# zijinxuxu/PDFNet

Hardware: AMD Instinct MI355X
Metric: train-step images/sec @256x256 RGB-D B=32 (higher is better)
Workload: dtype f32

## Files before the change

pdfnet_amd/csrc/winograd.hip:

```cpp
#include "common.h"
#include <cstdio>

int pdf_internal_batched_gemm(const float* A, const float* B, float* C, int batch, long gsA, long gsB, long gsC, int M, int N, int K, hipStream_t s);

template <bool FLIP>
__global__ __launch_bounds__(256) void wino_weight_kernel(const float* __restrict__ w, float* __restrict__ U, int Cout, int Cin) {
    const int N = FLIP ? Cin : Cout, K = FLIP ? Cout : Cin;
    const long total = (long)N * K;
    for (long i = blockIdx.x * 256L + threadIdx.x; i < total; i += (long)gridDim.x * 256) {
        const int n = (int)(i / K), k = (int)(i - (long)n * K);
        float g[3][3];
#pragma unroll
        for (int a = 0; a < 3; ++a)
#pragma unroll
            for (int b = 0; b < 3; ++b)
                g[a][b] = FLIP ? w[(((long)k * 3 + (2 - a)) * 3 + (2 - b)) * Cin + n] : w[(((long)n * 3 + a) * 3 + b) * Cin + k];
        float t[4][3];
#pragma unroll
        for (int b = 0; b < 3; ++b) {
            t[0][b] = g[0][b];
            t[1][b] = 0.5f * (g[0][b] + g[1][b] + g[2][b]);
            t[2][b] = 0.5f * (g[0][b] - g[1][b] + g[2][b]);
            t[3][b] = g[2][b];
        }
#pragma unroll
        for (int a = 0; a < 4; ++a) {
            const float u0 = t[a][0], u1 = 0.5f * (t[a][0] + t[a][1] + t[a][2]), u2 = 0.5f * (t[a][0] - t[a][1] + t[a][2]), u3 = t[a][2];
            U[(long)(a * 4 + 0) * total + i] = u0;
            U[(long)(a * 4 + 1) * total + i] = u1;
            U[(long)(a * 4 + 2) * total + i] = u2;
            U[(long)(a * 4 + 3) * total + i] = u3;
        }
    }
}

__global__ __launch_bounds__(256) void wino_input_kernel(const float* __restrict__ x, int ldx, float* __restrict__ V, int N, int H, int W, int C) {
    const int C4 = C >> 2, TW = W >> 1, TH = H >> 1;
    const long T = (long)N * TH * TW, total = T * C4;
    const long plane = T * C;
    for (long i = blockIdx.x * 256L + threadIdx.x; i < total; i += (long)gridDim.x * 256) {
        const long t = i / C4;
        const int c = (int)(i - t * C4) * 4;
        const int n = (int)(t / (TH * TW)), r = (int)(t - (long)n * TH * TW), ty = r / TW, tx = r - ty * TW;
        float4 d[4][4];
#pragma unroll
        for (int a = 0; a < 4; ++a) {
            const int iy = 2 * ty - 1 + a;
#pragma unroll
            for (int b = 0; b < 4; ++b) {
                const int ix = 2 * tx - 1 + b;
                d[a][b] = (iy >= 0 && iy < H && ix >= 0 && ix < W) ? *reinterpret_cast<const float4*>(x + (((long)n * H + iy) * W + ix) * ldx + c)
                                                                   : make_float4(0.f, 0.f, 0.f, 0.f);
            }
        }
        float4 s[4][4];
#pragma unroll
        for (int b = 0; b < 4; ++b) {
#define WSUB(p, q) make_float4(p.x - q.x, p.y - q.y, p.z - q.z, p.w - q.w)
#define WADD(p, q) make_float4(p.x + q.x, p.y + q.y, p.z + q.z, p.w + q.w)
            s[0][b] = WSUB(d[0][b], d[2][b]);
            s[1][b] = WADD(d[1][b], d[2][b]);
            s[2][b] = WSUB(d[2][b], d[1][b]);
            s[3][b] = WSUB(d[1][b], d[3][b]);
        }
#pragma unroll
        for (int a = 0; a < 4; ++a) {
            const float4 v0 = WSUB(s[a][0], s[a][2]), v1 = WADD(s[a][1], s[a][2]), v2 = WSUB(s[a][2], s[a][1]), v3 = WSUB(s[a][1], s[a][3]);
            float* o = V + t * C + c;
            *reinterpret_cast<float4*>(o + (long)(a * 4 + 0) * plane) = v0;
            *reinterpret_cast<float4*>(o + (long)(a * 4 + 1) * plane) = v1;
            *reinterpret_cast<float4*>(o + (long)(a * 4 + 2) * plane) = v2;
            *reinterpret_cast<float4*>(o + (long)(a * 4 + 3) * plane) = v3;
        }
    }
}

__global__ __launch_bounds__(256) void wino_output_kernel(const float* __restrict__ Mx, const float* __restrict__ bias, float* __restrict__ y, int ldy,
                                                          int N, int H, int W, int Co, int act, int accum) {
    const int C4 = Co >> 2, TW = W >> 1, TH = H >> 1;
    const long T = (long)N * TH * TW, total = T * C4;
    const long plane = T * Co;
    for (long i = blockIdx.x * 256L + threadIdx.x; i < total; i += (long)gridDim.x * 256) {
        const long t = i / C4;
        const int c = (int)(i - t * C4) * 4;
        const int n = (int)(t / (TH * TW)), r = (int)(t - (long)n * TH * TW), ty = r / TW, tx = r - ty * TW;
        float4 m[4][4];
        const float* p = Mx + t * Co + c;
#pragma unroll
        for (int a = 0; a < 4; ++a)
#pragma unroll
            for (int b = 0; b < 4; ++b) m[a][b] = *reinterpret_cast<const float4*>(p + (long)(a * 4 + b) * plane);
        float4 s[2][4];
#pragma unroll
        for (int b = 0; b < 4; ++b) {
            s[0][b] = WADD(WADD(m[0][b], m[1][b]), m[2][b]);
            s[1][b] = WSUB(WSUB(m[1][b], m[2][b]), m[3][b]);
        }
        const float4 bv = bias != nullptr ? *reinterpret_cast<const float4*>(bias + c) : make_float4(0.f, 0.f, 0.f, 0.f);
#pragma unroll
        for (int a = 0; a < 2; ++a) {
            float4 o[2];
            o[0] = WADD(WADD(s[a][0], s[a][1]), s[a][2]);
            o[1] = WSUB(WSUB(s[a][1], s[a][2]), s[a][3]);
#pragma unroll
            for (int b = 0; b < 2; ++b) {
                float4 v = WADD(o[b], bv);
                if (act == 1) v = make_float4(fmaxf(v.x, 0.f), fmaxf(v.y, 0.f), fmaxf(v.z, 0.f), fmaxf(v.w, 0.f));
                else if (act == 2) v = make_float4(v.x > 0.f ? v.x : 0.1f * v.x, v.y > 0.f ? v.y : 0.1f * v.y, v.z > 0.f ? v.z : 0.1f * v.z, v.w > 0.f ? v.w : 0.1f * v.w);
                float* q = y + (((long)n * H + 2 * ty + a) * W + 2 * tx + b) * ldy + c;
                if (accum) { const float4 e = *reinterpret_cast<const float4*>(q); v = WADD(v, e); }
                *reinterpret_cast<float4*>(q) = v;
            }
        }
    }
}
#undef WSUB
#undef WADD

template <bool FLIP, bool X3>
__global__ __launch_bounds__(256) void wino4_weight_kernel(const float* __restrict__ w, float* __restrict__ U, int Cout, int Cin) {
    const int N = FLIP ? Cin : Cout, K = FLIP ? Cout : Cin;
    const long total = (long)N * K;
    for (long i = blockIdx.x * 256L + threadIdx.x; i < total; i += (long)gridDim.x * 256) {
        const int n = (int)(i / K), k = (int)(i - (long)n * K);
        float g[3][3];
#pragma unroll
        for (int a = 0; a < 3; ++a)
#pragma unroll
            for (int b = 0; b < 3; ++b)
                g[a][b] = FLIP ? w[(((long)k * 3 + (2 - a)) * 3 + (2 - b)) * Cin + n] : w[(((long)n * 3 + a) * 3 + b) * Cin + k];
        float t[6][3];
#pragma unroll
        for (int b = 0; b < 3; ++b) {
            const float g0 = g[0][b], g1 = g[1][b], g2 = g[2][b];
            t[0][b] = g0 * 0.25f;
            t[1][b] = -(g0 + g1 + g2) * (1.f / 6.f);
            t[2][b] = -(g0 - g1 + g2) * (1.f / 6.f);
            t[3][b] = g0 * (1.f / 24.f) + g1 * (1.f / 12.f) + g2 * (1.f / 6.f);
            t[4][b] = g0 * (1.f / 24.f) - g1 * (1.f / 12.f) + g2 * (1.f / 6.f);
            t[5][b] = g2;
        }
#pragma unroll
        for (int a = 0; a < 6; ++a) {
            const float g0 = t[a][0], g1 = t[a][1], g2 = t[a][2];
            const float u[6] = {g0 * 0.25f, -(g0 + g1 + g2) * (1.f / 6.f), -(g0 - g1 + g2) * (1.f / 6.f),
                                g0 * (1.f / 24.f) + g1 * (1.f / 12.f) + g2 * (1.f / 6.f), g0 * (1.f / 24.f) - g1 * (1.f / 12.f) + g2 * (1.f / 6.f), g2};
#pragma unroll
            for (int b = 0; b < 6; ++b) {
                if constexpr (X3) {
                    unsigned h, m, l;
                    pdf_x3_split2(u[b], 0.f, h, m, l);
                    unsigned short* o = reinterpret_cast<unsigned short*>(U) + (long)(a * 6 + b) * total + i;
                    o[0] = (unsigned short)h; o[36 * total] = (unsigned short)m; o[72 * total] = (unsigned short)l;
                } else U[(long)(a * 6 + b) * total + i] = u[b];
            }
        }
    }
}
__device__ __forceinline__ void wino4_bt(float2 (&v)[6]) {
    const float2 d0 = v[0], d1 = v[1], d2 = v[2], d3 = v[3], d4 = v[4], d5 = v[5];
#define W4(e) make_float2(e(x), e(y))
#define E0(c) 4.f * d0.c - 5.f * d2.c + d4.c
#define E1(c) -4.f * (d1.c + d2.c) + d3.c + d4.c
#define E2(c) 4.f * (d1.c - d2.c) - d3.c + d4.c
#define E3(c) 2.f * (d3.c - d1.c) - d2.c + d4.c
#define E4(c) 2.f * (d1.c - d3.c) - d2.c + d4.c
#define E5(c) 4.f * d1.c - 5.f * d3.c + d5.c
    v[0] = W4(E0); v[1] = W4(E1); v[2] = W4(E2); v[3] = W4(E3); v[4] = W4(E4); v[5] = W4(E5);
#undef E0
#undef E1
#undef E2
#undef E3
#undef E4
#undef E5
}
template <bool X3>
__global__ __launch_bounds__(256) void wino4_input_kernel(const float* __restrict__ x, int ldx, float* __restrict__ V, int N, int H, int W, int C) {
    const int C2 = C >> 1, TW = W >> 2, TH = H >> 2;
    const long T = (long)N * TH * TW, total = T * C2;
    const long plane = T * C;
    for (long i = blockIdx.x * 256L + threadIdx.x; i < total; i += (long)gridDim.x * 256) {
        const long t = i / C2;
        const int c = (int)(i - t * C2) * 2;
        const int n = (int)(t / (TH * TW)), r = (int)(t - (long)n * TH * TW), ty = r / TW, tx = r - ty * TW;
        float2 d[6][6];
#pragma unroll
        for (int a = 0; a < 6; ++a) {
            const int iy = 4 * ty - 1 + a;
#pragma unroll
            for (int b = 0; b < 6; ++b) {
                const int ix = 4 * tx - 1 + b;
                d[a][b] = (iy >= 0 && iy < H && ix >= 0 && ix < W) ? *reinterpret_cast<const float2*>(x + (((long)n * H + iy) * W + ix) * ldx + c) : make_float2(0.f, 0.f);
            }
        }
#pragma unroll
        for (int b = 0; b < 6; ++b) {
            float2 col[6] = {d[0][b], d[1][b], d[2][b], d[3][b], d[4][b], d[5][b]};
            wino4_bt(col);
#pragma unroll
            for (int a = 0; a < 6; ++a) d[a][b] = col[a];
        }
        float* o = V + t * C + c;
#pragma unroll
        for (int a = 0; a < 6; ++a) {
            wino4_bt(d[a]);
#pragma unroll
            for (int b = 0; b < 6; ++b) {
                if constexpr (X3) pdf_x3_store2(reinterpret_cast<unsigned short*>(V), t * C + c + (long)(a * 6 + b) * plane, 36 * plane, d[a][b].x, d[a][b].y);
                else *reinterpret_cast<float2*>(o + (long)(a * 6 + b) * plane) = d[a][b];
            }
        }
    }
}
__global__ __launch_bounds__(256) void wino4_output_kernel(const float* __restrict__ Mx, const float* __restrict__ bias, float* __restrict__ y, int ldy,
                                                           int N, int H, int W, int Co, int act, int accum) {
    const int C2 = Co >> 1, TW = W >> 2, TH = H >> 2;
    const long T = (long)N * TH * TW, total = T * C2;
    const long plane = T * Co;
    for (long i = blockIdx.x * 256L + threadIdx.x; i < total; i += (long)gridDim.x * 256) {
        const long t = i / C2;
        const int c = (int)(i - t * C2) * 2;
        const int n = (int)(t / (TH * TW)), r = (int)(t - (long)n * TH * TW), ty = r / TW, tx = r - ty * TW;
        const float* p = Mx + t * Co + c;
        float2 s[4][6];
#pragma unroll
        for (int b = 0; b < 6; ++b) {
            float2 m[6];
#pragma unroll
            for (int a = 0; a < 6; ++a) m[a] = *reinterpret_cast<const float2*>(p + (long)(a * 6 + b) * plane);
#define O0(c) m[0].c + m[1].c + m[2].c + m[3].c + m[4].c
#define O1(c) m[1].c - m[2].c + 2.f * (m[3].c - m[4].c)
#define O2(c) m[1].c + m[2].c + 4.f * (m[3].c + m[4].c)
#define O3(c) m[1].c - m[2].c + 8.f * (m[3].c - m[4].c) + m[5].c
            s[0][b] = W4(O0); s[1][b] = W4(O1); s[2][b] = W4(O2); s[3][b] = W4(O3);
        }
        const float2 bv = bias != nullptr ? *reinterpret_cast<const float2*>(bias + c) : make_float2(0.f, 0.f);
#pragma unroll
        for (int a = 0; a < 4; ++a) {
            const float2* m = s[a];
            float2 o[4] = {W4(O0), W4(O1), W4(O2), W4(O3)};
#pragma unroll
            for (int b = 0; b < 4; ++b) {
                float2 v = make_float2(o[b].x + bv.x, o[b].y + bv.y);
                if (act == 1) v = make_float2(fmaxf(v.x, 0.f), fmaxf(v.y, 0.f));
                else if (act == 2) v = make_float2(v.x > 0.f ? v.x : 0.1f * v.x, v.y > 0.f ? v.y : 0.1f * v.y);
                float* q = y + (((long)n * H + 4 * ty + a) * W + 4 * tx + b) * ldy + c;
                if (accum) { const float2 e = *reinterpret_cast<const float2*>(q); v.x += e.x; v.y += e.y; }
                *reinterpret_cast<float2*>(q) = v;
            }
        }
#undef O0
#undef O1
#undef O2
#undef O3
#undef W4
    }
}

template <bool X3>
__global__ __launch_bounds__(256) void wino4_dy_kernel(const float* __restrict__ dy, int lddy, float* __restrict__ Yh, int N, int H, int W, int Co) {
    const int C2 = Co >> 1, TW = W >> 2, TH = H >> 2;
    const long T = (long)N * TH * TW, total = T * C2;
    const long plane = T * Co;
    for (long i = blockIdx.x * 256L + threadIdx.x; i < total; i += (long)gridDim.x * 256) {
        const long t = i / C2;
        const int c = (int)(i - t * C2) * 2;
        const int n = (int)(t / (TH * TW)), r = (int)(t - (long)n * TH * TW), ty = r / TW, tx = r - ty * TW;
        float2 d[4][4];
#pragma unroll
        for (int a = 0; a < 4; ++a)
#pragma unroll
            for (int b = 0; b < 4; ++b) d[a][b] = *reinterpret_cast<const float2*>(dy + (((long)n * H + 4 * ty + a) * W + 4 * tx + b) * lddy + c);
        float2 u[6][4];
#pragma unroll
        for (int b = 0; b < 4; ++b) {
#define A2(e) make_float2(e(x), e(y))
#define P0(k) d[0][b].k
#define P1(k) d[0][b].k + d[1][b].k + d[2][b].k + d[3][b].k
#define P2(k) d[0][b].k - d[1][b].k + d[2][b].k - d[3][b].k
#define P3(k) d[0][b].k + 2.f * d[1][b].k + 4.f * d[2][b].k + 8.f * d[3][b].k
#define P4(k) d[0][b].k - 2.f * d[1][b].k + 4.f * d[2][b].k - 8.f * d[3][b].k
#define P5(k) d[3][b].k
            u[0][b] = A2(P0); u[1][b] = A2(P1); u[2][b] = A2(P2); u[3][b] = A2(P3); u[4][b] = A2(P4); u[5][b] = A2(P5);
#undef P0
#undef P1
#undef P2
#undef P3
#undef P4
#undef P5
        }
        float* o = Yh + t * Co + c;
#pragma unroll
        for (int a = 0; a < 6; ++a) {
            const float2 e0 = u[a][0], e1 = u[a][1], e2 = u[a][2], e3 = u[a][3];
#define Q0(k) e0.k
#define Q1(k) e0.k + e1.k + e2.k + e3.k
#define Q2(k) e0.k - e1.k + e2.k - e3.k
#define Q3(k) e0.k + 2.f * e1.k + 4.f * e2.k + 8.f * e3.k
#define Q4(k) e0.k - 2.f * e1.k + 4.f * e2.k - 8.f * e3.k
#define Q5(k) e3.k
            const float2 q[6] = {A2(Q0), A2(Q1), A2(Q2), A2(Q3), A2(Q4), A2(Q5)};
#pragma unroll
            for (int b = 0; b < 6; ++b) {
                if constexpr (X3) pdf_x3_store2(reinterpret_cast<unsigned short*>(Yh), t * Co + c + (long)(a * 6 + b) * plane, 36 * plane, q[b].x, q[b].y);
                else *reinterpret_cast<float2*>(o + (long)(a * 6 + b) * plane) = q[b];
            }
#undef Q0
#undef Q1
#undef Q2
#undef Q3
#undef Q4
#undef Q5
#undef A2
        }
    }
}
__global__ __launch_bounds__(256) void wino4_slab_sum_kernel(float* __restrict__ slab, int splits, long total4) {
    for (long i = blockIdx.x * 256L + threadIdx.x; i < 36 * total4; i += (long)gridDim.x * 256) {
        const long p = i / total4, e = i - p * total4;
        float4* base = reinterpret_cast<float4*>(slab) + p * splits * total4 + e;
        float4 v = base[0];
        for (int y = 1; y < splits; ++y) { const float4 w = base[(long)y * total4]; v.x += w.x; v.y += w.y; v.z += w.z; v.w += w.w; }
        base[0] = v;
    }
}
__global__ __launch_bounds__(256) void wino4_wgrad_out_kernel(const float* __restrict__ slab, int splits, float* __restrict__ dw, int Co, int Ci, int accumulate) {
    const long total = (long)Co * Ci;
    for (long i = blockIdx.x * 256L + threadIdx.x; i < total; i += (long)gridDim.x * 256) {
        const int n = (int)(i / Ci), c = (int)(i - (long)n * Ci);
        float u[6][6];
#pragma unroll
        for (int p = 0; p < 36; ++p) u[p / 6][p % 6] = slab[(long)p * splits * total + i];
        {
        float t[3][6];
#pragma unroll
        for (int b = 0; b < 6; ++b) {
            t[0][b] = 0.25f * u[0][b] - (1.f / 6.f) * (u[1][b] + u[2][b]) + (1.f / 24.f) * (u[3][b] + u[4][b]);
            t[1][b] = (1.f / 6.f) * (u[2][b] - u[1][b]) + (1.f / 12.f) * (u[3][b] - u[4][b]);
            t[2][b] = -(1.f / 6.f) * (u[1][b] + u[2][b]) + (1.f / 6.f) * (u[3][b] + u[4][b]) + u[5][b];
        }
#pragma unroll
        for (int a = 0; a < 3; ++a) {
            const float g0 = 0.25f * t[a][0] - (1.f / 6.f) * (t[a][1] + t[a][2]) + (1.f / 24.f) * (t[a][3] + t[a][4]);
            const float g1 = (1.f / 6.f) * (t[a][2] - t[a][1]) + (1.f / 12.f) * (t[a][3] - t[a][4]);
            const float g2 = -(1.f / 6.f) * (t[a][1] + t[a][2]) + (1.f / 6.f) * (t[a][3] + t[a][4]) + t[a][5];
            float* o = dw + (((long)n * 3 + a) * 3) * Ci + c;
            if (accumulate) { o[0] += g0; o[Ci] += g1; o[2 * (long)Ci] += g2; }
            else { o[0] = g0; o[Ci] = g1; o[2 * (long)Ci] = g2; }
        }
        }
    }
}
int pdf_internal_batched_wgemm(const float* P, const float* Q, float* slab, int batch, long gsP, long gsQ, int M, int NI, int NJ, int splits, hipStream_t s);
int pdf_internal_x3_batched_gemm(const void* A3, long csA, const void* B3, long csB, float* C, int batch, long gsA, long gsB, long gsC,
                                 int M, int N, int K, int variant, int nprod, hipStream_t s);
int pdf_internal_x3_batched_wgemm(const void* P3, long csP, const void* Q3, long csQ, float* slab, int batch, long gsP, long gsQ,
                                  int M, int NI, int NJ, int splits, int variant, int nprod, hipStream_t s);
int pdf_internal_x3_mode();
static int x3_mode() { return pdf_internal_x3_mode() & 1; }
static int x3_nprod() {
    static const int v = getenv("PDF_X3_NPROD") ? atoi(getenv("PDF_X3_NPROD")) : 6;
    return v;
}
static int x3_minc() {
    static const int v = getenv("PDF_X3_MINC") ? atoi(getenv("PDF_X3_MINC")) : 256;
    return v;
}
static long x3_mint() {
    static const long v = getenv("PDF_X3_MINT") ? atol(getenv("PDF_X3_MINT")) : 2048;
    return v;
}
static bool wino_x3(long T, int C) { return x3_mode() != 0 && C >= x3_minc() && T >= x3_mint() && C % 32 == 0 && T % 32 == 0 && 73.0 * (double)T * C < 2147483000.0; }
static bool wino_x3_fits(long T, int C) { return x3_mode() != 0 && C % 32 == 0 && T % 32 == 0 && 73.0 * (double)T * C < 2147483000.0; }
int pdf_internal_colsum(const float* g, int ldg, int C, long R, float* out, int accumulate, float* ws, hipStream_t s);
long pdf_internal_colsum_ws(int C, long R);
static long wino_minpt();
static int wino_wgrad_splits(long T, int Co, int Ci) {
    const long tiles = 36L * cdiv(Co, 128) * cdiv(Ci, 128);
    long sp = (2304 + tiles - 1) / tiles;
    const long cap = T / 256 > 0 ? T / 256 : 1;
    if (sp > cap) sp = cap;
    return (int)(sp < 1 ? 1 : sp);
}
int pdf_internal_wino_wgrad_eligible(int N, int H, int W, int Cin, int Cout, int KH, int KW, int stride, int pad) {
    static const int on = getenv("PDF_WINOGRAD_WGRAD") ? atoi(getenv("PDF_WINOGRAD_WGRAD")) : 1;
    static const int minc = getenv("PDF_WINOGRAD_MINC") ? atoi(getenv("PDF_WINOGRAD_MINC")) : 128;
    if (!on || getenv("PDF_WINOGRAD") != nullptr && atoi(getenv("PDF_WINOGRAD")) == 0) return 0;
    if (KH != 3 || KW != 3 || stride != 1 || pad != 1 || H % 4 || W % 4) return 0;
    if (Cin % 16 || Cout % 16 || Cin < minc || Cout < 64) return 0;
    const long T = (long)N * (H / 4) * (W / 4);
    if (T % 16 != 0 || 36 * T < wino_minpt()) return 0;
    if ((double)T * (Cin > Cout ? Cin : Cout) * 4.0 > 4.0e9) return 0;
    return 1;
}
long pdf_internal_wino_wgrad_workspace(int N, int H, int W, int Cin, int Cout) {
    const long T = (long)N * (H / 4) * (W / 4);
    const bool x3 = wino_x3(T, Cin) && wino_x3_fits(T, Cout);
    return (x3 ? 54L : 36L) * T * Cin + (x3 ? 54L : 36L) * T * Cout + 36L * wino_wgrad_splits(T, Cout, Cin) * Cout * Cin + pdf_internal_colsum_ws(Cout, (long)N * H * W) + 64;
}
int pdf_internal_conv3x3_winograd_wgrad(const float* x, int ldx, const float* dy, int lddy, float* dw, float* db, float* ws,
                                        int N, int H, int W, int Cin, int Cout, int accumulate, const float* v_cached, hipStream_t s) {
    const long T = (long)N * (H / 4) * (W / 4);
    const bool x3 = wino_x3(T, Cin) && wino_x3_fits(T, Cout);
    if (v_cached != nullptr && wino_x3(T, Cin) != x3) v_cached = nullptr;
    const long per = x3 ? 54L : 36L;
    float* V = ws;
    float* Yh = V + per * T * Cin;
    float* slab = Yh + per * T * Cout;
    const int splits = wino_wgrad_splits(T, Cout, Cin);
    float* cws = slab + 36L * splits * Cout * Cin;
    if (v_cached == nullptr) {
        if (x3) hipLaunchKernelGGL((wino4_input_kernel<true>), dim3(grid_for(T * (Cin / 2), 256, 256 * 32)), dim3(256), 0, s, x, ldx, V, N, H, W, Cin);
        else hipLaunchKernelGGL((wino4_input_kernel<false>), dim3(grid_for(T * (Cin / 2), 256, 256 * 32)), dim3(256), 0, s, x, ldx, V, N, H, W, Cin);
    }
    if (x3) hipLaunchKernelGGL((wino4_dy_kernel<true>), dim3(grid_for(T * (Cout / 2), 256, 256 * 32)), dim3(256), 0, s, dy, lddy, Yh, N, H, W, Cout);
    else hipLaunchKernelGGL((wino4_dy_kernel<false>), dim3(grid_for(T * (Cout / 2), 256, 256 * 32)), dim3(256), 0, s, dy, lddy, Yh, N, H, W, Cout);
    PDF_LAUNCH_CHECK();
    const float* Vq = v_cached != nullptr ? v_cached : V;
    const int used = x3 ? pdf_internal_x3_batched_wgemm(Yh, 36L * T * Cout, Vq, 36L * T * Cin, slab, 36, T * Cout, T * Cin, (int)T, Cout, Cin, splits, -1, x3_nprod(), s)
                        : pdf_internal_batched_wgemm(Yh, Vq, slab, 36, T * Cout, T * Cin, (int)T, Cout, Cin, splits, s);
    if (used <= 0) return used < 0 ? used : PDF_E_BADARG;
    if (used > 1) hipLaunchKernelGGL(wino4_slab_sum_kernel, dim3(grid_for(36L * Cout * Cin / 4)), dim3(256), 0, s, slab, used, (long)Cout * Cin / 4);
    hipLaunchKernelGGL(wino4_wgrad_out_kernel, dim3(grid_for((long)Cout * Cin)), dim3(256), 0, s, slab, used, dw, Cout, Cin, accumulate);
    PDF_LAUNCH_CHECK();
    if (db != nullptr) return pdf_internal_colsum(dy, lddy, Cout, (long)N * H * W, db, accumulate, cws, s);
    return 0;
}

static int wino_mode() {
    static const int v = getenv("PDF_WINOGRAD") ? atoi(getenv("PDF_WINOGRAD")) : 4;
    return v;
}
static long wino_minpt() {
    static const long v = getenv("PDF_WINOGRAD_MINPT") ? atol(getenv("PDF_WINOGRAD_MINPT")) : 16384;
    return v;
}
int pdf_internal_wino_tile(int N, int H, int W, int Ck, int Cn, int flip) {
    static const int f4 = getenv("PDF_WINOGRAD_F4") ? atoi(getenv("PDF_WINOGRAD_F4")) : 15;
    const int mode = wino_mode();
    if (mode == 0) return 0;
    const int bit = ((Ck > 256 || Cn > 256) ? 4 : 1) << (flip ? 1 : 0);
    for (int m = (mode == 4 && (f4 & bit)) ? 4 : 2; m >= 2; m -= 2) {
        if (H % m || W % m) continue;
        const long T = (long)N * (H / m) * (W / m), P = (m + 2) * (m + 2);
        if (P * T < wino_minpt()) continue;
        if ((double)T * (Ck > Cn ? Ck : Cn) * 4.0 > 4.0e9) continue;
        return m;
    }
    return 0;
}
long pdf_internal_wino_workspace(int N, int H, int W, int Ck, int Cn, int flip) {
    const int m = pdf_internal_wino_tile(N, H, W, Ck, Cn, flip);
    if (m == 0) return 0;
    const long T = (long)N * (H / m) * (W / m), P = (m + 2) * (m + 2);
    if (m == 4 && (flip ? (wino_x3_fits(T, Ck) && (Ck >= x3_minc() || Cn >= x3_minc())) : wino_x3(T, Ck))) return 54L * Cn * Ck + 54L * T * Ck + P * T * Cn;
    return P * Cn * Ck + P * T * Ck + P * T * Cn;
}
long pdf_internal_wino_v_offset(int N, int H, int W, int Ck, int Cn) {
    if (pdf_internal_wino_tile(N, H, W, Ck, Cn, 0) != 4) return -1;
    return (wino_x3((long)N * (H / 4) * (W / 4), Ck) ? 54L : 36L) * Cn * Ck;
}
int pdf_internal_wino_eligible(int N, int H, int W, int Ck, int Cn, int KH, int KW, int stride, int pad, int flip) {
    static const int minc = getenv("PDF_WINOGRAD_MINC") ? atoi(getenv("PDF_WINOGRAD_MINC")) : 128;
    if (KH != 3 || KW != 3 || stride != 1 || pad != 1) return 0;
    if (Ck % 16 != 0 || Cn % 16 != 0 || Ck < minc || Cn < 64) return 0;
    return pdf_internal_wino_tile(N, H, W, Ck, Cn, flip) != 0;
}
int pdf_internal_conv3x3_winograd(const float* x, int ldx, const float* w, const float* bias, float* y, int ldy, float* ws,
                                  int N, int H, int W, int Ck, int Cn, int act, int accum, int flip, const float* v_shared, hipStream_t s) {
    const int m = pdf_internal_wino_tile(N, H, W, Ck, Cn, flip);
    const long T = (long)N * (H / m) * (W / m), P = (m + 2) * (m + 2);
    const bool x3 = m == 4 && (flip ? (wino_x3_fits(T, Ck) && (Ck >= x3_minc() || Cn >= x3_minc())) : wino_x3(T, Ck));
    const long upl = x3 ? 54L * Cn * Ck : P * Cn * Ck, vpl = x3 ? 54L * T * Ck : P * T * Ck;
    float* U = ws;
    const float* V = U + upl;
    float* Mx = ws + upl + vpl;
    const int gw = grid_for((long)Cn * Ck);
    if (m == 4) {
        if (x3 && flip) hipLaunchKernelGGL((wino4_weight_kernel<true, true>), dim3(gw), dim3(256), 0, s, w, U, Ck, Cn);
        else if (x3) hipLaunchKernelGGL((wino4_weight_kernel<false, true>), dim3(gw), dim3(256), 0, s, w, U, Cn, Ck);
        else if (flip) hipLaunchKernelGGL((wino4_weight_kernel<true, false>), dim3(gw), dim3(256), 0, s, w, U, Ck, Cn);
        else hipLaunchKernelGGL((wino4_weight_kernel<false, false>), dim3(gw), dim3(256), 0, s, w, U, Cn, Ck);
        if (v_shared != nullptr && !flip) V = v_shared;
        else if (x3) hipLaunchKernelGGL((wino4_input_kernel<true>), dim3(grid_for(T * (Ck / 2), 256, 256 * 32)), dim3(256), 0, s, x, ldx, U + upl, N, H, W, Ck);
        else hipLaunchKernelGGL((wino4_input_kernel<false>), dim3(grid_for(T * (Ck / 2), 256, 256 * 32)), dim3(256), 0, s, x, ldx, U + upl, N, H, W, Ck);
    } else {
        if (flip) hipLaunchKernelGGL((wino_weight_kernel<true>), dim3(gw), dim3(256), 0, s, w, U, Ck, Cn);
        else hipLaunchKernelGGL((wino_weight_kernel<false>), dim3(gw), dim3(256), 0, s, w, U, Cn, Ck);
        hipLaunchKernelGGL(wino_input_kernel, dim3(grid_for(T * (Ck / 4), 256, 256 * 32)), dim3(256), 0, s, x, ldx, U + upl, N, H, W, Ck);
    }
    PDF_LAUNCH_CHECK();
    if (x3) {
        if (int rc = pdf_internal_x3_batched_gemm(V, 36L * T * Ck, U, 36L * Cn * Ck, Mx, 36, T * Ck, (long)Cn * Ck, T * Cn, (int)T, Cn, Ck, -1, x3_nprod(), s)) return rc;
    } else if (int rc = pdf_internal_batched_gemm(V, U, Mx, (int)P, T * Ck, (long)Cn * Ck, T * Cn, (int)T, Cn, Ck, s)) return rc;
    if (m == 4) hipLaunchKernelGGL(wino4_output_kernel, dim3(grid_for(T * (Cn / 2), 256, 256 * 32)), dim3(256), 0, s, Mx, bias, y, ldy, N, H, W, Cn, act, accum);
    else hipLaunchKernelGGL(wino_output_kernel, dim3(grid_for(T * (Cn / 4), 256, 256 * 32)), dim3(256), 0, s, Mx, bias, y, ldy, N, H, W, Cn, act, accum);
    PDF_LAUNCH_CHECK();
    return 0;
}
```

Measured before the change: 724.3.

## Fuse Winograd F4 wgrad split-K slab reduction into output transform kernel

Merges the separate split-K slab summation kernel into the weight-gradient output transform. Each 576-thread block reduces 36 Winograd planes for 64 weight elements into shared memory, then 192 threads apply the inverse transform, one row per thread. This removes one launch and the write-back and re-read of the reduced slab, but only a third of the threads do the transform stage. It also assumes Co*Ci is a multiple of 4 for the float4 loads.

Measured after the change: 725.2 (median of 5 runs). No clear change (+0.1%).

```diff
diff --git a/pdfnet_amd/csrc/winograd.hip b/pdfnet_amd/csrc/winograd.hip
--- a/pdfnet_amd/csrc/winograd.hip
+++ b/pdfnet_amd/csrc/winograd.hip
@@ -315,41 +315,45 @@
         }
     }
 }
-__global__ __launch_bounds__(256) void wino4_slab_sum_kernel(float* __restrict__ slab, int splits, long total4) {
-    for (long i = blockIdx.x * 256L + threadIdx.x; i < 36 * total4; i += (long)gridDim.x * 256) {
-        const long p = i / total4, e = i - p * total4;
-        float4* base = reinterpret_cast<float4*>(slab) + p * splits * total4 + e;
-        float4 v = base[0];
-        for (int y = 1; y < splits; ++y) { const float4 w = base[(long)y * total4]; v.x += w.x; v.y += w.y; v.z += w.z; v.w += w.w; }
-        base[0] = v;
-    }
-}
-__global__ __launch_bounds__(256) void wino4_wgrad_out_kernel(const float* __restrict__ slab, int splits, float* __restrict__ dw, int Co, int Ci, int accumulate) {
+#define WO_E 64
+__global__ __launch_bounds__(576) void wino4_wgrad_out_kernel(const float* __restrict__ slab, int splits, float* __restrict__ dw, int Co, int Ci, int accumulate) {
+    __shared__ float4 us[36][WO_E / 4];
     const long total = (long)Co * Ci;
-    for (long i = blockIdx.x * 256L + threadIdx.x; i < total; i += (long)gridDim.x * 256) {
-        const int n = (int)(i / Ci), c = (int)(i - (long)n * Ci);
-        float u[6][6];
-#pragma unroll
-        for (int p = 0; p < 36; ++p) u[p / 6][p % 6] = slab[(long)p * splits * total + i];
-        {
-        float t[3][6];
-#pragma unroll
-        for (int b = 0; b < 6; ++b) {
-            t[0][b] = 0.25f * u[0][b] - (1.f / 6.f) * (u[1][b] + u[2][b]) + (1.f / 24.f) * (u[3][b] + u[4][b]);
-            t[1][b] = (1.f / 6.f) * (u[2][b] - u[1][b]) + (1.f / 12.f) * (u[3][b] - u[4][b]);
-            t[2][b] = -(1.f / 6.f) * (u[1][b] + u[2][b]) + (1.f / 6.f) * (u[3][b] + u[4][b]) + u[5][b];
-        }
-#pragma unroll
-        for (int a = 0; a < 3; ++a) {
-            const float g0 = 0.25f * t[a][0] - (1.f / 6.f) * (t[a][1] + t[a][2]) + (1.f / 24.f) * (t[a][3] + t[a][4]);
-            const float g1 = (1.f / 6.f) * (t[a][2] - t[a][1]) + (1.f / 12.f) * (t[a][3] - t[a][4]);
-            const float g2 = -(1.f / 6.f) * (t[a][1] + t[a][2]) + (1.f / 6.f) * (t[a][3] + t[a][4]) + t[a][5];
-            float* o = dw + (((long)n * 3 + a) * 3) * Ci + c;
-            if (accumulate) { o[0] += g0; o[Ci] += g1; o[2 * (long)Ci] += g2; }
-            else { o[0] = g0; o[Ci] = g1; o[2 * (long)Ci] = g2; }
-        }
-        }
-    }
+    const int tid = threadIdx.x;
+    {
+        const int p = tid >> 4, q = tid & 15;
+        const long e0 = blockIdx.x * (long)WO_E + q * 4;
+        float4 v = make_float4(0.f, 0.f, 0.f, 0.f);
+        if (e0 < total) {
+            const float4* base = reinterpret_cast<const float4*>(slab + (long)p * splits * total + e0);
+            const long total4 = total / 4;
+            v = base[0];
+            for (int y = 1; y < splits; ++y) { const float4 w = base[(long)y * total4]; v.x += w.x; v.y += w.y; v.z += w.z; v.w += w.w; }
+        }
+        us[p][q] = v;
+    }
+    __syncthreads();
+    if (tid >= 192) return;
+    const int a = tid >> 6, el = tid & 63;
+    const long i = blockIdx.x * (long)WO_E + el;
+    if (i >= total) return;
+    const int n = (int)(i / Ci), c = (int)(i - (long)n * Ci);
+    const float* uf = reinterpret_cast<const float*>(&us[0][0]) + el;
+    float t[6];
+#pragma unroll
+    for (int b = 0; b < 6; ++b) {
+#define U(r) uf[((r) * 6 + b) * WO_E]
+        if (a == 0) t[b] = 0.25f * U(0) - (1.f / 6.f) * (U(1) + U(2)) + (1.f / 24.f) * (U(3) + U(4));
+        else if (a == 1) t[b] = (1.f / 6.f) * (U(2) - U(1)) + (1.f / 12.f) * (U(3) - U(4));
+        else t[b] = -(1.f / 6.f) * (U(1) + U(2)) + (1.f / 6.f) * (U(3) + U(4)) + U(5);
+#undef U
+    }
+    const float g0 = 0.25f * t[0] - (1.f / 6.f) * (t[1] + t[2]) + (1.f / 24.f) * (t[3] + t[4]);
+    const float g1 = (1.f / 6.f) * (t[2] - t[1]) + (1.f / 12.f) * (t[3] - t[4]);
+    const float g2 = -(1.f / 6.f) * (t[1] + t[2]) + (1.f / 6.f) * (t[3] + t[4]) + t[5];
+    float* o = dw + (((long)n * 3 + a) * 3) * Ci + c;
+    if (accumulate) { o[0] += g0; o[Ci] += g1; o[2 * (long)Ci] += g2; }
+    else { o[0] = g0; o[Ci] = g1; o[2 * (long)Ci] = g2; }
 }
 int pdf_internal_batched_wgemm(const float* P, const float* Q, float* slab, int batch, long gsP, long gsQ, int M, int NI, int NJ, int splits, hipStream_t s);
 int pdf_internal_x3_batched_gemm(const void* A3, long csA, const void* B3, long csB, float* C, int batch, long gsA, long gsB, long gsC,
@@ -420,8 +424,7 @@
     const int used = x3 ? pdf_internal_x3_batched_wgemm(Yh, 36L * T * Cout, Vq, 36L * T * Cin, slab, 36, T * Cout, T * Cin, (int)T, Cout, Cin, splits, -1, x3_nprod(), s)
                         : pdf_internal_batched_wgemm(Yh, Vq, slab, 36, T * Cout, T * Cin, (int)T, Cout, Cin, splits, s);
     if (used <= 0) return used < 0 ? used : PDF_E_BADARG;
-    if (used > 1) hipLaunchKernelGGL(wino4_slab_sum_kernel, dim3(grid_for(36L * Cout * Cin / 4)), dim3(256), 0, s, slab, used, (long)Cout * Cin / 4);
-    hipLaunchKernelGGL(wino4_wgrad_out_kernel, dim3(grid_for((long)Cout * Cin)), dim3(256), 0, s, slab, used, dw, Cout, Cin, accumulate);
+    hipLaunchKernelGGL(wino4_wgrad_out_kernel, dim3(cdiv((long)Cout * Cin, (long)WO_E)), dim3(576), 0, s, slab, used, dw, Cout, Cin, accumulate);
     PDF_LAUNCH_CHECK();
     if (db != nullptr) return pdf_internal_colsum(dy, lddy, Cout, (long)N * H * W, db, accumulate, cws, s);
     return 0;
```
